# kawshik8/GAN-Image-Captioning

Hardware: AMD Instinct MI355X
Metric: captions/sec (G+D train step) (higher is better)
Workload: dtype bf16; 1 GPU; cfg2: adversarial G+D step, batch 64/GPU, 224x224 images, caption len 20, V=10000, E=H=512, 1-layer LSTM G, CNN-seq D (R=64,F=900), ResNet-50-shaped encoder, --conditional-gan 1; global_batch=64, caption_len=20, image_size=224, vocab=10000, conditional_gan=1, encoder=resnet50, step_impl=fused, parallelism=dp1

## Files before the change

gan-image-captioning_amd/_lib.py:

```python
from __future__ import annotations

import ctypes as C
import os

import torch

from . import build as _build

MAX_LAYERS = 4
MAX_CONVS = 8
F32, BF16 = 0, 1
LOSS_TYPES = {"standard": 0, "JS": 1, "KL": 2, "hinge": 3, "tv": 4, "rsgan": 5}

c_float_p = C.POINTER(C.c_float)
c_void_p = C.c_void_p


class DecoderDims(C.Structure):
    _fields_ = [(n, C.c_int32) for n in ("B", "L", "V", "E", "H", "NL", "dtype")]


class DecoderParams(C.Structure):
    _fields_ = [("embed", c_void_p), ("w_ih", c_void_p * MAX_LAYERS), ("w_hh", c_void_p * MAX_LAYERS),
                ("b_ih", c_void_p * MAX_LAYERS), ("b_hh", c_void_p * MAX_LAYERS), ("w_out", c_void_p), ("b_out", c_void_p)]
# ... 217 lines not shown
    "gic_repack_conv_weight": (C.c_int, [c_void_p, c_void_p, C.c_int, C.c_int, C.c_int, C.c_int, C.c_int, C.c_int, C.c_int, c_void_p]),
    "gic_conv2d_bn_in": (C.c_int, [c_void_p, c_void_p, C.c_int, c_void_p, c_void_p, C.c_float, c_void_p, c_void_p, c_void_p, C.c_int,
                         C.c_int] + [C.c_int] * 9 + [c_void_p]),
    "gic_conv1x1_res_in": (C.c_int, [c_void_p, c_void_p, C.c_int, c_void_p, c_void_p, c_void_p, c_void_p, C.c_int, c_void_p, c_void_p, C.c_float,
                           c_void_p, c_void_p, c_void_p, c_void_p, C.c_int, C.c_int, C.c_int, C.c_int, C.c_int, C.c_int, C.c_int, c_void_p]),
    "gic_conv1x1_bn_in_stats": (C.c_int, [c_void_p, c_void_p, C.c_int, c_void_p, c_void_p, C.c_float, c_void_p, c_void_p, C.c_int, C.c_int, C.c_int64,
                                C.c_int, C.c_int, c_void_p]),
    "gic_conv_b2b": (C.c_int, [c_void_p, c_void_p, C.c_int, c_void_p, c_void_p, c_void_p, c_void_p, C.c_int, c_void_p, c_void_p, c_void_p, c_void_p,
                     C.c_int, c_void_p, c_void_p, C.c_float, c_void_p, c_void_p, c_void_p, c_void_p, C.c_int, C.c_int, C.c_int64, C.c_int, C.c_int,
                     c_void_p]),
    "gic_conv_b2b_supported": (C.c_int, [C.c_int, C.c_int64, C.c_int, C.c_int]),
    "gic_conv2d": (C.c_int, [c_void_p, c_void_p, c_void_p, c_void_p, C.c_int, C.c_int] + [C.c_int] * 9 + [c_void_p]),
    "gic_bn_act": (C.c_int, [c_void_p] * 12 + [C.c_int, C.c_float, C.c_int, c_void_p, C.c_int, C.c_int64, C.c_int, c_void_p]),
    "gic_bn_relu_maxpool": (C.c_int, [c_void_p] * 6 + [C.c_int, C.c_float, c_void_p, C.c_int, C.c_int, C.c_int, C.c_int, C.c_int, c_void_p]),
    "gic_avgpool": (C.c_int, [c_void_p, c_void_p, C.c_int, C.c_int, C.c_int, C.c_int, c_void_p]),
    "gic_bn_running_update": (C.c_int, [c_void_p, C.c_int, c_void_p]),
    "gic_bn1d_fwd": (C.c_int, [c_void_p] * 5 + [C.c_int, C.c_float, C.c_float, c_void_p, c_void_p, c_void_p, C.c_int, C.c_int, c_void_p]),
    "gic_bn1d_bwd": (C.c_int, [c_void_p] * 4 + [C.c_int, c_void_p, c_void_p, c_void_p, C.c_int, C.c_int, c_void_p]),
    "gic_colsum": (C.c_int, [c_void_p, C.c_int, C.c_int64, C.c_int64, C.c_int64, c_void_p, C.c_int, c_void_p]),
    "gic_gan_losses": (C.c_int, [C.c_int, c_void_p, c_void_p, c_void_p, C.c_int64, c_void_p, c_void_p, c_void_p, c_void_p,
                                 c_void_p, c_void_p, c_void_p]),
    "gic_xent": (C.c_int, [c_void_p, C.c_int, C.c_int64, C.c_int32, c_void_p, c_void_p, c_void_p, c_void_p, c_void_p]),
    "gic_xent_seq": (C.c_int, [c_void_p, C.c_int, C.c_int64, C.c_int32, c_void_p, C.c_int64, c_void_p, C.c_int64, C.c_float, c_void_p, c_void_p,
                               c_void_p, c_void_p, c_void_p, c_void_p, c_void_p, c_void_p]),
    "gic_rollout_rewards": (C.c_int, [c_void_p, c_void_p, c_void_p, C.c_int, C.c_int, C.c_int, C.c_int, c_void_p]),
    "gic_cider_d": (C.c_int, [c_void_p, C.c_int64, c_void_p, c_void_p, C.c_int32, C.c_int32, c_void_p, C.c_int64, c_void_p, c_void_p,
                              C.c_int32, C.c_int32, C.c_int32, C.c_int32, c_void_p, c_void_p, C.c_int64, C.c_float, C.c_int32, c_void_p,
                              c_void_p]),
    "gic_caption_overlap": (C.c_int, [c_void_p, C.c_int64, c_void_p, c_void_p, C.c_int32, C.c_int32, c_void_p, C.c_int64, c_void_p, c_void_p,
                                      C.c_int32, C.c_int32, C.c_int32, C.c_int32, C.c_int32, c_void_p, c_void_p, c_void_p, c_void_p]),
# ... 60 lines not shown
```

gan-image-captioning_amd/csrc/encoder.hip:

```cpp
#include "../../include/gicap.h"
#include "kernels.h"
#include "bn_fold.h"
#include "conv_b2b.h"

namespace gic {
namespace {

template <typename TA, int PX>
__global__ __launch_bounds__(256) void pack_image_kernel(const float* __restrict__ img, TA* __restrict__ out, int N, int S, int pad, int Hp, int Wp) {
  const int groups = Wp / PX;
  const int total = N * Hp * groups;
  for (int i = blockIdx.x * blockDim.x + threadIdx.x; i < total; i += gridDim.x * blockDim.x) {
    const int gq = i % groups, t = i / groups;
    const int hp = t % Hp, n = t / Hp;
    const int h = hp - pad;
    const bool hok = h >= 0 && h < S;
    const int hc = min(max(h, 0), S - 1);
    float v[PX][3];
#pragma unroll
    for (int q = 0; q < PX; ++q) {
      const int w = gq * PX + q - pad;
      const int wc = min(max(w, 0), S - 1);
#pragma unroll
      for (int c = 0; c < 3; ++c) v[q][c] = img[(((long)n * 3 + c) * S + hc) * S + wc];
// ... 54 lines not shown
  shift = b.beta[c] - mean * scale;
}

__device__ __forceinline__ void stage_coeffs(float* coef, const BnSrc& b, int C, float inv_count) {
  for (int c = threadIdx.x; c < C; c += blockDim.x) {
    float sc, sh;
    bn_coeffs(b, c, C, inv_count, sc, sh);
    coef[c] = sc;
    coef[C + c] = sh;
  }
}

template <typename TA> struct Vec16 { static constexpr int N = 16 / sizeof(TA); };

template <typename TA, bool RES>
__global__ __launch_bounds__(1024) void bn_act_kernel(const TA* __restrict__ y, BnSrc by, const TA* __restrict__ res, BnSrc br,
                                                      float inv_count, int relu, TA* __restrict__ out, long rows, int C) {
  extern __shared__ __attribute__((aligned(16))) float coef[];
  constexpr int VN = Vec16<TA>::N;
  stage_coeffs(coef, by, C, inv_count);
  if (RES) stage_coeffs(coef + 2 * C, br, C, inv_count);
  __syncthreads();
  const int cv = C / VN;
  const long i0 = (long)blockIdx.x * blockDim.x + threadIdx.x;
  const int c0 = (int)(i0 % cv) * VN;
  float sc[VN], sh[VN], rs[VN], rh[VN];
#pragma unroll
  for (int k = 0; k < VN; ++k) {
    sc[k] = coef[c0 + k]; sh[k] = coef[C + c0 + k];
    rs[k] = RES ? coef[2 * C + c0 + k] : 0.f; rh[k] = RES ? coef[3 * C + c0 + k] : 0.f;
  }
  const long R = (long)gridDim.x * blockDim.x / cv;
  for (long r = i0 / cv; r < rows; r += 4 * R) {
    TA yv[4][VN], rv[4][VN];
    long o[4];
#pragma unroll
    for (int u = 0; u < 4; ++u) {
      const long ru = r + u * R;
      o[u] = (ru < rows ? ru : r) * C + c0;
      *(uint4*)yv[u] = *(const uint4*)(y + o[u]);
      if (RES) *(uint4*)rv[u] = *(const uint4*)(res + o[u]);
    }
#pragma unroll
    for (int u = 0; u < 4; ++u) {
      TA ov[VN];
#pragma unroll
      for (int k = 0; k < VN; ++k) {
        float v = to_f32<TA>(yv[u][k]) * sc[k] + sh[k];
        if (RES) v += to_f32<TA>(rv[u][k]) * rs[k] + rh[k];
        if (relu) v = fmaxf(v, 0.f);
        ov[k] = from_f32<TA>(v);
      }
      if (r + u * R < rows) *(uint4*)(out + o[u]) = *(const uint4*)ov;
    }
  }
}

template <typename TA>
__global__ __launch_bounds__(1024) void bn_relu_maxpool_kernel(const TA* __restrict__ y, BnSrc by, float inv_count, TA* __restrict__ out,
                                                                int N, int H, int W, int C, int Ho, int Wo) {
  extern __shared__ __attribute__((aligned(16))) float coef[];
  constexpr int VN = Vec16<TA>::N;
  stage_coeffs(coef, by, C, inv_count);
  __syncthreads();
  const int cv = C / VN;
  const long i0 = (long)blockIdx.x * blockDim.x + threadIdx.x;
  const int c0 = (int)(i0 % cv) * VN;
  float sc[VN], sh[VN];
#pragma unroll
// ... 33 lines not shown
  for (long i = (long)blockIdx.x * blockDim.x + threadIdx.x; i < total; i += (long)gridDim.x * blockDim.x) {
    const int c = (int)(i % C);
    const long n = i / C;
    const TA* xp = x + n * HW * C + c;
    float s = 0.f;
    int p = 0;
    for (; p + 7 <= HW; p += 7) {
      float v[7];
#pragma unroll
      for (int q = 0; q < 7; ++q) v[q] = to_f32<TA>(xp[(long)(p + q) * C]);
#pragma unroll
      for (int q = 0; q < 7; ++q) s += v[q];
    }
    for (; p < HW; ++p) s += to_f32<TA>(xp[(long)p * C]);
    out[i] = from_f32<TA>(s / (float)HW);
  }
}

__global__ void bn_running_update_kernel(const gic_bn_running_desc* __restrict__ table, int nlayers) {
  const int l = blockIdx.x;
  if (l >= nlayers) return;
  const gic_bn_running_desc d = table[l];
  const float inv = 1.f / d.count;
  const float unbias = d.count > 1.f ? d.count / (d.count - 1.f) : 1.f;
  for (int c = blockIdx.y * blockDim.x + threadIdx.x; c < d.C; c += blockDim.x * gridDim.y) {
    float s1 = 0.f, s2 = 0.f;
    for (int r = 0; r < d.nrep; ++r) { s1 += d.stats[(long)r * 2 * d.C + c]; s2 += d.stats[(long)r * 2 * d.C + d.C + c]; }
    const float mean = s1 * inv;
    const float var = fmaxf(s2 * inv - mean * mean, 0.f);
    d.running_mean[c] = (1.f - d.momentum) * d.running_mean[c] + d.momentum * mean;
// ... 59 lines not shown
  sg = bn1d_colsum(sg, red, r, c);
  sb = bn1d_colsum(sb, red, r, c);
  if (!live) return;
  if (r == 0) { dgamma[e] = sg; dbeta[e] = sb; }
  const float k = gamma[e] * invstd[e];
  const float invB = 1.f / (float)B;
  for (int b = r; b < B; b += 16) {
    const float d = dy[(long)b * E + e];
    dx[(long)b * E + e] = training ? k * (d - invB * (sb + xhat[(long)b * E + e] * sg)) : k * d;
  }
}

inline int grid1d(long total, int cap = 4096) {
  long g = (total + 255) / 256;
  return (int)(g < 1 ? 1 : (g > cap ? cap : g));
}
inline int bn_act_grid(long total) {
  long g = (total + 1023) / 1024;
  return (int)(g < 1 ? 1 : (g > 512 ? 512 : g));
}
inline int grid_periodic(long total, int period, int cap = 4096) {
  int g = grid1d(total, cap);
  const int mult = period > 256 ? period / 256 : 1;
  g = (g + mult - 1) / mult * mult;
  return g;
}

BnSrc make_src(const float* stats, int nrep, const float* gamma, const float* beta, const float* rm, const float* rv) {
  BnSrc s;
  s.stats = stats; s.nrep = nrep < 1 ? 1 : nrep; s.gamma = gamma; s.beta = beta; s.run_mean = rm; s.run_var = rv;
  return s;
}

GemmDesc conv_desc(const void* in, const void* w, void* out, float* stats, int stats_nrep, int dtype, int N, int H, int W, int Cin, int Cout,
// ... 123 lines not shown
  if (dtype != DT_BF16) return GIC_ERR_UNSUPPORTED;
  GemmDesc g = conv_desc(in, w, out, stats, stats_nrep, dtype, N, H, W, Cin, Cout, 1, 1, 1, 0);
  bn_on_load(g, in_stats, in_nrep, in_gamma, in_beta, count);
  g.res = res; g.res_stats = res_stats; g.res_nrep = res_nrep; g.res_gamma = res_gamma; g.res_beta = res_beta; g.res_inv_count = 1.f / count;
  g.out_wb = block_out;
  return gemm(g, (hipStream_t)stream);
}

int gic_bn_act(const void* y, const float* stats, const float* gamma, const float* beta, const float* run_mean, const float* run_var,
               const void* res, const float* res_stats, const float* res_gamma, const float* res_beta, const float* res_run_mean,
               const float* res_run_var, int stats_nrep, float count, int relu, void* out, int dtype, int64_t rows, int C, void* stream) {
  GIC_CHECK_ARG(y && out && gamma && beta && (stats || run_mean) && rows > 0 && count > 0, "bn_act: bad argument");
  const BnSrc by = make_src(stats, stats_nrep, gamma, beta, run_mean, run_var);
  const BnSrc br = make_src(res_stats, stats_nrep, res_gamma, res_beta, res_run_mean, res_run_var);
  GIC_CHECK_ARG(C % 8 == 0 && (C & (C - 1)) == 0, "bn_act: C must be a power of two >= 8 (got %d)", C);
  const size_t lds = (size_t)4 * C * sizeof(float);
  const int cv = C / (dtype == DT_F32 ? 4 : 8);
  const long total = rows * cv;
  int grid = bn_act_grid(total);
  {
    int step = cv, t = 1024;
    while (t) { const int m = step % t; step = t; t = m; }
    const int mult = cv / step;
    grid = (grid + mult - 1) / mult * mult;
    static const bool fit = getenv("GIC_BN_ACT_NO_FIT") == nullptr;
    if (fit && total > 4 * 1024) {
      const long rr = (rows + 3) / 4;
      long g = (rr * cv + 1023) / 1024;
      g = (g + mult - 1) / mult * mult;
      if (g <= 512) grid = (int)g;
    }
  }
  const hipStream_t st = (hipStream_t)stream;
  if (dtype == DT_F32) {
    if (res) hipLaunchKernelGGL((bn_act_kernel<float, true>), dim3(grid), dim3(1024), lds, st, (const float*)y, by, (const float*)res, br, 1.f / count, relu, (float*)out, (long)rows, C);
    else hipLaunchKernelGGL((bn_act_kernel<float, false>), dim3(grid), dim3(1024), lds, st, (const float*)y, by, (const float*)res, br, 1.f / count, relu, (float*)out, (long)rows, C);
  } else {
    if (res) hipLaunchKernelGGL((bn_act_kernel<bf16_t, true>), dim3(grid), dim3(1024), lds, st, (const bf16_t*)y, by, (const bf16_t*)res, br, 1.f / count, relu, (bf16_t*)out, (long)rows, C);
    else hipLaunchKernelGGL((bn_act_kernel<bf16_t, false>), dim3(grid), dim3(1024), lds, st, (const bf16_t*)y, by, (const bf16_t*)res, br, 1.f / count, relu, (bf16_t*)out, (long)rows, C);
  }
  GIC_CHECK_LAUNCH("bn_act");
  return GIC_OK;
}

int gic_bn_relu_maxpool(const void* y, const float* stats, const float* gamma, const float* beta, const float* run_mean,
                        const float* run_var, int stats_nrep, float count, void* out, int dtype, int N, int H, int W, int C, void* stream) {
  GIC_CHECK_ARG(y && out && gamma && beta && (stats || run_mean) && C % 8 == 0, "bn_relu_maxpool: bad argument");
  const int Ho = (H + 2 - 3) / 2 + 1, Wo = (W + 2 - 3) / 2 + 1;
  const BnSrc by = make_src(stats, stats_nrep, gamma, beta, run_mean, run_var);
  const size_t lds = (size_t)2 * C * sizeof(float);
  const int cv = C / (dtype == DT_F32 ? 4 : 8);
  const long total = (long)N * Ho * Wo * cv;
  GIC_CHECK_ARG((long)N * Ho * Wo < (1l << 31), "bn_relu_maxpool: too many output pixels");
  int grid = (int)((total + 1023) / 1024);
// ... 11 lines not shown
  GIC_CHECK_LAUNCH("bn_relu_maxpool");
  return GIC_OK;
}

int gic_avgpool(const void* x, void* out, int dtype, int N, int HW, int C, void* stream) {
  GIC_CHECK_ARG(x && out && N > 0 && HW > 0 && C > 0, "avgpool: bad argument");
  const long total = (long)N * C;
  if (dtype == DT_F32)
    hipLaunchKernelGGL((avgpool_kernel<float>), dim3(grid1d(total)), dim3(256), 0, (hipStream_t)stream, (const float*)x, (float*)out, N, HW, C);
  else
    hipLaunchKernelGGL((avgpool_kernel<bf16_t>), dim3(grid1d(total)), dim3(256), 0, (hipStream_t)stream, (const bf16_t*)x, (bf16_t*)out, N, HW, C);
  GIC_CHECK_LAUNCH("avgpool");
  return GIC_OK;
}

int gic_bn_running_update(const gic_bn_running_desc* table_dev, int nlayers, void* stream) {
  GIC_CHECK_ARG(table_dev && nlayers > 0, "bn_running_update: bad argument");
  hipLaunchKernelGGL(bn_running_update_kernel, dim3(nlayers, 8), dim3(256), 0, (hipStream_t)stream, table_dev, nlayers);
  GIC_CHECK_LAUNCH("bn_running_update");
  return GIC_OK;
}

int gic_bn1d_fwd(const float* x, const float* gamma, const float* beta, float* running_mean, float* running_var, int training,
                 float momentum, float eps, float* y, float* xhat, float* invstd, int B, int E, void* stream) {
  GIC_CHECK_ARG(x && gamma && beta && running_mean && running_var && y && xhat && invstd && B > 0 && E > 0, "bn1d_fwd: bad argument");
  hipLaunchKernelGGL(bn1d_fwd_kernel, dim3(cdiv(E, 16)), dim3(256), 0, (hipStream_t)stream, x, gamma, beta, running_mean, running_var,
                     training, momentum, eps, y, xhat, invstd, B, E);
  GIC_CHECK_LAUNCH("bn1d_fwd");
  return GIC_OK;
}
// ... 16 lines not shown
```

gan-image-captioning_amd/encoder_engine.py:

```python
from __future__ import annotations

import ctypes as C
import os
from typing import Dict, List, Optional, Tuple

import torch

from . import _lib as L
from . import engine
from .engine import ptr, stream_ptr

AVAILABLE = True
STATS_REPLICAS = 8


def _check(status, what):
    L.check(status, what)


class _NullCtx:
    def __enter__(self):
        return self

    def __exit__(self, *exc):
# ... 51 lines not shown
        off = 0
        for s in self.steps:
            s.stats_off = off
            off += 2 * s.cout * STATS_REPLICAS
        self.stats_len = off
        self._wkey = None
        self._bufs: Dict[Tuple[int, int], dict] = {}
        self._graphs: Dict[tuple, "torch.cuda.CUDAGraph"] = {}
        self._warm: set = set()
        self.fuse_in = not os.environ.get("GIC_NO_FUSED_BN_IN")
        self.fuse_res = os.environ.get("GIC_FUSED_RES_IN", "1") != "0"
        self.res_min_rows = int(os.environ.get("GIC_RES_IN_MIN_ROWS", "50000"))
        self.res_max_cout = int(os.environ.get("GIC_RES_IN_MAX_COUT", "128"))
        self.fuse_b2b = not os.environ.get("GIC_NO_CONV_B2B")
        self.b2b_only = int(os.environ.get("GIC_B2B_ONLY", "0"))
        self._nrep = {}
        self._det = False
        self.use_graph = not os.environ.get("GIC_NO_GRAPH")
        self.pending_tracked = 0
        self.conv_trace = None

    def sync_counters(self) -> None:
        if self.pending_tracked:
            for s in self.steps:
                s.bn.num_batches_tracked += self.pending_tracked
            self.pending_tracked = 0

    def _pack_weights(self, dev) -> None:
        key = (self.trunk._ptr_epoch, tuple(s.conv.weight._version for s in self.steps))
        if key == self._wkey:
# ... 198 lines not shown

    def _bn_args(self, s: Optional[_ConvStep], stats: Optional[torch.Tensor], training: bool):
        if s is None:
            return (None,) * 5
        g, b = ptr(s.bn.weight.detach()), ptr(s.bn.bias.detach())
        if training:
            return (stats.data_ptr() + 4 * s.stats_off, g, b, None, None)
        return (None, g, b, ptr(s.bn.running_mean), ptr(s.bn.running_var))

    def _bn_act(self, s, y, out, stats, training, rows, relu=True, res=None, res_step=None):
        a = self._bn_args(s, stats, training)
        r = self._bn_args(res_step, stats, training)
        _check(L.load().gic_bn_act(ptr(y), *a, ptr(res), *r, self._nrep[s.name], float(rows), int(relu), ptr(out), self.dtype, rows, s.cout, stream_ptr()),
               "gic_bn_act " + s.name)

    def forward(self, images: torch.Tensor, training: bool) -> torch.Tensor:
        engine.require_gpu(images)
        if images.dim() != 4 or images.shape[1] != 3 or images.shape[2] != images.shape[3] or images.dtype != torch.float32:
            raise ValueError(f"images must be float32 [N,3,S,S], got {tuple(images.shape)} {images.dtype}")
        N, S = images.shape[0], images.shape[2]
        if S % 2:
            raise ValueError("image size must be even")
        dev = images.device
        lib = L.load()
        self._det = engine.deterministic()
        self._cur = self._bkey(N, S)
        self._pack_weights(dev)
        b = self._buffers(N, S, dev)
        _check(lib.gic_pack_image(ptr(images.contiguous()), ptr(b["xin"]), self.dtype, N, S, 3, S + 6, stream_ptr()), "gic_pack_image")
        self._launch_trunk(b, N, S, training)
        if training:
            self.pending_tracked += 1
        return b["feat"]

    def last_map(self, N: int, S: int) -> torch.Tensor:
        return self._bufs[self._bkey(N, S)]["blocks"][-1]["out"]

    def _launch_trunk(self, b: dict, N: int, S: int, training: bool) -> None:
        if not self.use_graph:
            return self._run_trunk(b, N, S, training)
        key = (N, S, bool(training), self._det, self._wkey)
        g = self._graphs.get(key)
        if g is not None:
            g.replay()
        elif key not in self._warm:
            self._warm.add(key)
            self._run_trunk(b, N, S, training)
        else:
            self._graphs.clear()
            g = torch.cuda.CUDAGraph()
            try:
                with engine.capture_guard(), torch.cuda.graph(g, capture_error_mode="thread_local"):
                    self._run_trunk(b, N, S, training)
            except Exception as exc:
                import warnings
                warnings.warn(f"hipGraph capture of the trunk forward failed ({exc}); falling back to eager launches")
                self.use_graph = False
                torch.cuda.synchronize()
                return self._run_trunk(b, N, S, training)
            self._graphs[key] = g
            g.replay()

    def _run_trunk(self, b: dict, N: int, S: int, training: bool) -> None:
        lib = L.load()
        stats = b["stats"] if training else None
        if training:
            b["stats"].zero_()
        rows = b["rows"]
        self._conv(self.stem, b["xin"], b["y0"], stats, N, S + 6, S + 6, cin=4, kw=8, pad=0)
        h = b["y0"].shape[1]
        a = self._bn_args(self.stem, stats, training)
        _check(lib.gic_bn_relu_maxpool(ptr(b["y0"]), *a, self._nrep[self.stem.name], float(rows[self.stem.name]), ptr(b["x0"]), self.dtype, N, h, h, 64, stream_ptr()),
               "gic_bn_relu_maxpool")
        x = b["x0"]
        pend = None
        fuse_res = training and self.fuse_res and self.dtype != L.F32 and not self._det

        def flush():
            nonlocal pend
            if pend is not None:
                last, ylast, res, res_step, rows_, out = pend
                self._bn_act(last, ylast, out, stats, training, rows_, res=res, res_step=res_step)
                pend = None

        pend_b2b = None
        for bi, (blk, e) in enumerate(zip(self.blocks, b["blocks"])):
            c1, c2, c3, ds = blk["c1"], blk["c2"], blk["c3"], blk["ds"]
            hin, ho = e["hin"], e["hout"]
            nxt = self.blocks[bi + 1] if bi + 1 < len(self.blocks) else None
            b2b = False
            if blk["kind"] == "basic":
                flush()
                self._conv(c1, x, e["y1"], stats, N, hin, hin)
                self._bn_relu_conv(c1, e["y1"], e["z1"], c2, e["y2"], stats, training, N, ho, ho, rows[c1.name])
                last, ylast = c2, e["y2"]
            else:
                if pend_b2b is not None:
                    self._conv_b2b(pend_b2b, c1, e["y1"], stats)
                    pend_b2b = None
                elif pend is None or not self._conv1_res_in(pend, c1, e["y1"], stats, N, hin, hin):
                    flush()
                    self._conv(c1, x, e["y1"], stats, N, hin, hin)
                pend = None
                self._bn_relu_conv(c1, e["y1"], e["z1"], c2, e["y2"], stats, training, N, hin, hin, rows[c1.name])
                b2b = self._b2b_ok(blk, nxt, rows[c3.name], training) and self._conv3_stats_only(blk, e["y2"], stats, rows[c2.name], rows[c3.name])
                blk["b2b"] = bool(b2b)
                if not b2b:
                    self._bn_relu_conv(c2, e["y2"], e["z2"], c3, e["y3"], stats, training, N, ho, ho, rows[c2.name])
                last, ylast = c3, e["y3"]
            if ds is not None:
                self._conv(ds, x, e["yd"], stats, N, hin, hin)
                res, res_step = e["yd"], ds
            else:
                res, res_step = x, None
            if blk["kind"] != "basic" and b2b:
                pend_b2b = (c2, e["y2"], c3, res, res_step, rows[c3.name], e["out"])
            elif fuse_res and blk["kind"] != "basic":
                pend = (last, ylast, res, res_step, rows[last.name], e["out"])
            else:
                self._bn_act(last, ylast, e["out"], stats, training, rows[last.name], res=res, res_step=res_step)
            x = e["out"]
        flush()
        ho = x.shape[1]
        _check(lib.gic_avgpool(ptr(x), ptr(b["feat"]), self.dtype, N, ho * ho, x.shape[3], stream_ptr()), "gic_avgpool")
        if training:
            _check(lib.gic_bn_running_update(ptr(b["table"]), len(self.steps), stream_ptr()), "gic_bn_running_update")

    def replay(self, s: _ConvStep, xi, yo, stats, N: int, H: int, W: int, kw: dict, prev=None) -> None:
        if prev is not None and prev[0] == "b2b":
            self._conv_b2b(prev[1], s, yo, stats)
        elif prev is not None and prev[0] == "b2bstats":
            if not self._conv3_stats_only(prev[1], prev[2], stats, prev[3], prev[4]):
                raise RuntimeError("statistics-only conv3 refused for " + s.name)
        elif prev is not None and prev[0] == "res":
            if s.fused_in and self._conv1_res_in(prev[1], s, yo, stats, N, H, W):
                return
            self._conv(s, xi, yo, stats, N, H, W, **kw)
        elif prev is not None and s.fused_in:
            p, yp, rows_p = prev
# ... 156 lines not shown
```

gan-image-captioning_amd/generator.py:

```python
from __future__ import annotations

import math
from typing import List, Optional

import torch
import torch.nn as nn

from . import engine
from .trunk import ResNetTrunk, encoder_head_bwd, encoder_head_fwd


def _compute_dtype(args) -> int:
    return engine.parse_dtype(getattr(args, "compute_dtype", "bf16"))


class _SeedStream:

    def __init__(self):
        self._n = 0

    rank = 0

    def reset(self, n: int = 0) -> None:
        self._n = int(n)
# ... 520 lines not shown
                                   self.linear.weight, self.linear.bias, self.bn.weight, self.bn.bias,
                                   self.bn.running_mean, self.bn.running_var)
        return out, fmap.view(fmap.shape[0], -1, fmap.shape[-1])

    def prefetch_trunk(self, images, training: bool, after, mark=None, want_map: bool = False) -> None:
        if getattr(self, "_s_pre", None) is None:
            self._s_pre = torch.cuda.Stream(device=images.device)
        s = self._s_pre
        with engine.on_stream(s):
            s.wait_event(after)
            busy, self._busy = getattr(self, "_busy", None), None
            if busy is not None:
                s.wait_event(busy)
            if mark is not None:
                mark("trunk prefetch start [s_pre]", s)
            feats = self.trunk_features(images, training).clone()
            fmap = self.resnet._plan.last_map(images.shape[0], images.shape[2]).clone() if want_map else None
            done = s.record_event()
            if mark is not None:
                mark("trunk prefetch done [s_pre]", s)
        images.record_stream(s)
        self._pre = (images, bool(training), feats, done, fmap)

    def take_trunk(self, images, training: bool, stream):
        pre, self._pre = getattr(self, "_pre", None), None
        if pre is not None:
            stream.wait_event(pre[3])
            if pre[0] is images and pre[1] == bool(training):
                pre[2].record_stream(stream)
                return pre[2]
        busy = getattr(self, "_busy", None)
# ... 7 lines not shown
        pre, self._pre = getattr(self, "_pre", None), None
        if pre is not None:
            stream.wait_event(pre[3])
            if pre[0] is images and pre[1] == bool(training) and pre[4] is not None:
                pre[2].record_stream(stream)
                pre[4].record_stream(stream)
                return pre[2], pre[4]
        busy = getattr(self, "_busy", None)
        if busy is not None:
            stream.wait_event(busy)
        feats = self.trunk_features(images, training).clone()
        fmap = self.resnet._plan.last_map(images.shape[0], images.shape[2]).clone()
        self._busy = stream.record_event()
        return feats, fmap

    def trunk_features(self, images, training: bool):
        return self.resnet(images, _compute_dtype(self.args), training)

    def forward_fused(self, images, training: bool, trunk_feats=None):
        dt = _compute_dtype(self.args)
        feats = trunk_feats if trunk_feats is not None else self.resnet(images, dt, training)
        out, self._saved = encoder_head_fwd(dt, feats, self.linear.weight.detach(), self.linear.bias.detach(),
                                            self.bn.weight.detach(), self.bn.bias.detach(), self.bn.running_mean,
                                            self.bn.running_var, training, self.bn.momentum, self.bn.eps)
        return out

    def backward_fused(self, d_feat):
        grads = (self.linear.weight.grad, self.linear.bias.grad, self.bn.weight.grad, self.bn.bias.grad)
        encoder_head_bwd(_compute_dtype(self.args), self._saved, self.linear.weight.detach(), self.bn.weight.detach(), d_feat,
                         grads=grads)
        self._saved = None

# ... 96 lines not shown
```

gan-image-captioning_amd/trunk.py:

```python
from __future__ import annotations

from typing import Dict, List, Tuple

import torch
import torch.nn as nn

ARCHS = {
    "resnet18": ("basic", (2, 2, 2, 2), (64, 128, 256, 512), 1),
    "resnet50": ("bottleneck", (3, 4, 6, 3), (64, 128, 256, 512), 4),
}


class _ConvParams(nn.Module):
    def __init__(self, cin, cout, k, stride, pad):
        super().__init__()
        self.cin, self.cout, self.k, self.stride, self.pad = cin, cout, k, stride, pad
        w = torch.empty(cout, cin, k, k)
        nn.init.kaiming_normal_(w, mode="fan_out", nonlinearity="relu")
        self.weight = nn.Parameter(w)


class _BNParams(nn.Module):
    def __init__(self, c):
        super().__init__()
# ... 45 lines not shown
        self._plan = None
        self._ptr_epoch = 0
        self.register_load_state_dict_post_hook(lambda module, incompatible: module._bump_ptr_epoch())

    def _bump_ptr_epoch(self) -> None:
        self._ptr_epoch += 1

    def _apply(self, fn, *args, **kwargs):
        out = super()._apply(fn, *args, **kwargs)
        self._ptr_epoch += 1
        return out

    def stages(self) -> List[nn.Sequential]:
        return [getattr(self, str(i)) for i in (4, 5, 6, 7)]

    def forward(self, images: torch.Tensor, dtype: int, training=None) -> torch.Tensor:
        from . import encoder_engine
        if self._plan is None or self._plan.dtype != dtype:
            self._plan = encoder_engine.TrunkPlan(self, dtype)
        return self._plan.forward(images, self.training if training is None else training)

    def state_dict(self, *a, **k):
        if self._plan is not None:
            self._plan.sync_counters()
        return super().state_dict(*a, **k)


def encoder_head_fwd(dtype, feat, weight, bias, gamma, beta, running_mean, running_var, training, momentum, eps):
    from . import encoder_engine
    return encoder_engine.head_fwd(dtype, feat, weight, bias, gamma, beta, running_mean, running_var, training, momentum, eps)


def encoder_head_bwd(dtype, saved, weight, gamma, d_out, grads=None):
    from . import encoder_engine
    return encoder_engine.head_bwd(dtype, saved, weight, gamma, d_out, grads=grads)
# ... 1 lines not shown
```

include/gicap.h:

```cpp
#ifndef GICAP_H_
#define GICAP_H_

#include <stdint.h>

#ifdef __cplusplus
extern "C" {
#endif

#define GIC_ABI_VERSION 5
#define GIC_MAX_LAYERS 4
#define GIC_MAX_CONVS 8

enum gic_status {
  GIC_STATUS_OK = 0,
  GIC_STATUS_INVALID_ARG = -1,
  GIC_STATUS_UNSUPPORTED = -2,
  GIC_STATUS_LAUNCH = -3,
  GIC_STATUS_WORKSPACE = -4
};
enum gic_dtype { GIC_F32 = 0, GIC_BF16 = 1 };
enum gic_loss_type {
  GIC_LOSS_STANDARD = 0, GIC_LOSS_JS = 1, GIC_LOSS_KL = 2, GIC_LOSS_HINGE = 3, GIC_LOSS_TV = 4, GIC_LOSS_RSGAN = 5
};

// ... 403 lines not shown
int gic_conv1x1_bn_in_stats(const void* in, const float* in_stats, int in_nrep, const float* in_gamma, const float* in_beta, float in_count,
                            const void* w, float* stats, int stats_nrep, int dtype, int64_t rows, int Cin, int Cout, void* stream);
int gic_conv_b2b(const void* y2, const float* stats2, int nrep2, const float* gamma2, const float* beta2, const void* w3, const float* stats3,
                 int nrep3, const float* gamma3, const float* beta3, const void* res, const float* res_stats, int res_nrep,
                 const float* res_gamma, const float* res_beta, float count, void* block_out, const void* w1n, void* y1n, float* stats1,
                 int nrep1, int dtype, int64_t rows, int C2, int C1N, void* stream);
int gic_conv_b2b_supported(int dtype, int64_t rows, int C2, int C1N);
int gic_bn_act(const void* y, const float* stats, const float* gamma, const float* beta, const float* run_mean,
               const float* run_var, const void* res, const float* res_stats, const float* res_gamma, const float* res_beta,
               const float* res_run_mean, const float* res_run_var, int stats_nrep, float count, int relu, void* out, int dtype,
               int64_t rows, int C, void* stream);
int gic_bn_relu_maxpool(const void* y, const float* stats, const float* gamma, const float* beta, const float* run_mean,
                        const float* run_var, int stats_nrep, float count, void* out, int dtype, int N, int H, int W, int C,
                        void* stream);
int gic_avgpool(const void* x, void* out, int dtype, int N, int HW, int C, void* stream);
typedef struct gic_bn_running_desc {
  const float* stats;
  float* running_mean;
  float* running_var;
  float count;
  float momentum;
  int32_t C;
  int32_t nrep;
} gic_bn_running_desc;
int gic_bn_running_update(const gic_bn_running_desc* table_dev, int nlayers, void* stream);
int gic_bn1d_fwd(const float* x, const float* gamma, const float* beta, float* running_mean, float* running_var, int training,
                 float momentum, float eps, float* y, float* xhat, float* invstd, int B, int E, void* stream);
int gic_bn1d_bwd(const float* dy, const float* xhat, const float* invstd, const float* gamma, int training, float* dx,
                 float* dgamma, float* dbeta, int B, int E, void* stream);
int gic_colsum(const void* A, int dtype, int64_t lda, int64_t rows, int64_t cols, float* out, int accumulate, void* stream);
// ... 42 lines not shown
```

Baseline: 26930 captions/s.

## Fuse final BN-activation with average pooling and retile bn_act kernel

Adds a bn_act_avgpool kernel that applies the last block's BN, residual and ReLU, stages the result in LDS, and reduces it to pooled features in the same pass. Writing the full feature map becomes optional when the caller does not need it. This removes a separate avgpool pass and its reread of the map. The generic bn_act kernel is also reworked to use 256-thread blocks over 64-channel groups, computing only per-group coefficients and issuing the next loads before the current tile is processed. The cost is new plumbing through trunk, generator and graph keys, plus a fallback path when LDS is too small.

```diff
diff --git a/gan-image-captioning_amd/_lib.py b/gan-image-captioning_amd/_lib.py
--- a/gan-image-captioning_amd/_lib.py
+++ b/gan-image-captioning_amd/_lib.py
@@ -255,6 +255,7 @@
     "gic_bn_act": (C.c_int, [c_void_p] * 12 + [C.c_int, C.c_float, C.c_int, c_void_p, C.c_int, C.c_int64, C.c_int, c_void_p]),
     "gic_bn_relu_maxpool": (C.c_int, [c_void_p] * 6 + [C.c_int, C.c_float, c_void_p, C.c_int, C.c_int, C.c_int, C.c_int, C.c_int, c_void_p]),
     "gic_avgpool": (C.c_int, [c_void_p, c_void_p, C.c_int, C.c_int, C.c_int, C.c_int, c_void_p]),
+    "gic_bn_act_avgpool": (C.c_int, [c_void_p] * 12 + [C.c_int, C.c_float, C.c_int, c_void_p, c_void_p, C.c_int, C.c_int, C.c_int, C.c_int, c_void_p]),
     "gic_bn_running_update": (C.c_int, [c_void_p, C.c_int, c_void_p]),
     "gic_bn1d_fwd": (C.c_int, [c_void_p] * 5 + [C.c_int, C.c_float, C.c_float, c_void_p, c_void_p, c_void_p, C.c_int, C.c_int, c_void_p]),
     "gic_bn1d_bwd": (C.c_int, [c_void_p] * 4 + [C.c_int, c_void_p, c_void_p, c_void_p, C.c_int, C.c_int, c_void_p]),
diff --git a/gan-image-captioning_amd/csrc/encoder.hip b/gan-image-captioning_amd/csrc/encoder.hip
--- a/gan-image-captioning_amd/csrc/encoder.hip
+++ b/gan-image-captioning_amd/csrc/encoder.hip
@@ -92,45 +92,65 @@
 template <typename TA> struct Vec16 { static constexpr int N = 16 / sizeof(TA); };
 
 template <typename TA, bool RES>
-__global__ __launch_bounds__(1024) void bn_act_kernel(const TA* __restrict__ y, BnSrc by, const TA* __restrict__ res, BnSrc br,
-                                                      float inv_count, int relu, TA* __restrict__ out, long rows, int C) {
-  extern __shared__ __attribute__((aligned(16))) float coef[];
+__device__ __forceinline__ TA bn_act_elem(TA yv, TA rv, float sc, float sh, float rs, float rh, int relu) {
+  float v = to_f32<TA>(yv) * sc + sh;
+  if (RES) v += to_f32<TA>(rv) * rs + rh;
+  if (relu) v = fmaxf(v, 0.f);
+  return from_f32<TA>(v);
+}
+
+constexpr int kBnActCG = 64;
+template <typename TA, bool RES>
+__global__ __launch_bounds__(256) void bn_act_kernel(const TA* __restrict__ y, BnSrc by, const TA* __restrict__ res, BnSrc br,
+                                                     float inv_count, int relu, TA* __restrict__ out, long rows, int C, int CG) {
+  __shared__ float coef[4 * kBnActCG];
   constexpr int VN = Vec16<TA>::N;
-  stage_coeffs(coef, by, C, inv_count);
-  if (RES) stage_coeffs(coef + 2 * C, br, C, inv_count);
-  __syncthreads();
-  const int cv = C / VN;
-  const long i0 = (long)blockIdx.x * blockDim.x + threadIdx.x;
-  const int c0 = (int)(i0 % cv) * VN;
-  float sc[VN], sh[VN], rs[VN], rh[VN];
-#pragma unroll
-  for (int k = 0; k < VN; ++k) {
-    sc[k] = coef[c0 + k]; sh[k] = coef[C + c0 + k];
-    rs[k] = RES ? coef[2 * C + c0 + k] : 0.f; rh[k] = RES ? coef[3 * C + c0 + k] : 0.f;
-  }
-  const long R = (long)gridDim.x * blockDim.x / cv;
-  for (long r = i0 / cv; r < rows; r += 4 * R) {
-    TA yv[4][VN], rv[4][VN];
-    long o[4];
+  const int lanes = CG / VN, slots = 256 / lanes, groups = C / CG;
+  const int g = blockIdx.x % groups;
+  const long chunk = blockIdx.x / groups, nchunk = gridDim.x / groups;
+  const int cl = (threadIdx.x % lanes) * VN, slot = threadIdx.x / lanes;
+  const long col = (long)g * CG + cl;
+  {
+    const int t = threadIdx.x;
+    float a, b;
+    if (t < CG) {
+      bn_coeffs(by, g * CG + t, C, inv_count, a, b);
+      coef[t] = a; coef[CG + t] = b;
+    } else if (RES && t < 2 * CG) {
+      bn_coeffs(br, g * CG + t - CG, C, inv_count, a, b);
+      coef[2 * CG + t - CG] = a; coef[3 * CG + t - CG] = b;
+    }
+  }
+  long r = chunk * (4 * slots) + slot;
+  TA yv[4][VN], rv[4][VN];
+  long o[4];
+  auto issue = [&](long r_) {
 #pragma unroll
     for (int u = 0; u < 4; ++u) {
-      const long ru = r + u * R;
-      o[u] = (ru < rows ? ru : r) * C + c0;
+      const long ru = r_ + (long)u * slots;
+      o[u] = (ru < rows ? ru : rows - 1) * C + col;
       *(uint4*)yv[u] = *(const uint4*)(y + o[u]);
       if (RES) *(uint4*)rv[u] = *(const uint4*)(res + o[u]);
     }
+  };
+  issue(r);
+  __syncthreads();
+  float sc[VN], sh[VN], rs[VN], rh[VN];
+#pragma unroll
+  for (int k = 0; k < VN; ++k) {
+    sc[k] = coef[cl + k]; sh[k] = coef[CG + cl + k];
+    rs[k] = RES ? coef[2 * CG + cl + k] : 0.f; rh[k] = RES ? coef[3 * CG + cl + k] : 0.f;
+  }
+  while (r < rows) {
 #pragma unroll
     for (int u = 0; u < 4; ++u) {
       TA ov[VN];
 #pragma unroll
-      for (int k = 0; k < VN; ++k) {
-        float v = to_f32<TA>(yv[u][k]) * sc[k] + sh[k];
-        if (RES) v += to_f32<TA>(rv[u][k]) * rs[k] + rh[k];
-        if (relu) v = fmaxf(v, 0.f);
-        ov[k] = from_f32<TA>(v);
-      }
-      if (r + u * R < rows) *(uint4*)(out + o[u]) = *(const uint4*)ov;
-    }
+      for (int k = 0; k < VN; ++k) ov[k] = bn_act_elem<TA, RES>(yv[u][k], rv[u][k], sc[k], sh[k], rs[k], rh[k], relu);
+      if (r + (long)u * slots < rows) *(uint4*)(out + o[u]) = *(const uint4*)ov;
+    }
+    r += nchunk * (4 * slots);
+    if (r < rows) issue(r);
   }
 }
 
@@ -194,6 +214,80 @@
     }
     for (; p < HW; ++p) s += to_f32<TA>(xp[(long)p * C]);
     out[i] = from_f32<TA>(s / (float)HW);
+  }
+}
+
+constexpr int kPoolCG = 64;
+template <typename TA, bool RES>
+__global__ __launch_bounds__(256) void bn_act_avgpool_kernel(const TA* __restrict__ y, BnSrc by, const TA* __restrict__ res, BnSrc br,
+                                                              float inv_count, int relu, TA* __restrict__ out, TA* __restrict__ pooled,
+                                                              int HW, int C) {
+  extern __shared__ __attribute__((aligned(16))) float pool_lds[];
+  constexpr int VN = Vec16<TA>::N, CG = kPoolCG, CV = CG / VN, SLOTS = 256 / CV;
+  float* coef = pool_lds;
+  TA* tile = (TA*)(pool_lds + 4 * CG);
+  const int groups = C / CG;
+  const int g = blockIdx.x % groups;
+  const long n = blockIdx.x / groups;
+  const int cl = (threadIdx.x % CV) * VN;
+  const int slot = threadIdx.x / CV;
+  const long base = n * HW * C + g * CG + cl;
+  TA yv[2][VN], rv[2][VN];
+  auto issue = [&](int p0) {
+#pragma unroll
+    for (int u = 0; u < 2; ++u) {
+      const int p = min(p0 + slot + u * SLOTS, HW - 1);
+      *(uint4*)yv[u] = *(const uint4*)(y + base + (long)p * C);
+      if (RES) *(uint4*)rv[u] = *(const uint4*)(res + base + (long)p * C);
+    }
+  };
+  {
+    const int t = threadIdx.x;
+    float a, b;
+    if (t < CG) {
+      bn_coeffs(by, g * CG + t, C, inv_count, a, b);
+      coef[t] = a; coef[CG + t] = b;
+    } else if (RES && t < 2 * CG) {
+      bn_coeffs(br, g * CG + t - CG, C, inv_count, a, b);
+      coef[2 * CG + t - CG] = a; coef[3 * CG + t - CG] = b;
+    }
+  }
+  issue(0);
+  __syncthreads();
+  float sc[VN], sh[VN], rs[VN], rh[VN];
+#pragma unroll
+  for (int k = 0; k < VN; ++k) {
+    sc[k] = coef[cl + k]; sh[k] = coef[CG + cl + k];
+    rs[k] = RES ? coef[2 * CG + cl + k] : 0.f; rh[k] = RES ? coef[3 * CG + cl + k] : 0.f;
+  }
+  for (int p0 = 0; p0 < HW; p0 += 2 * SLOTS) {
+#pragma unroll
+    for (int u = 0; u < 2; ++u) {
+      const int p = p0 + slot + u * SLOTS;
+      TA ov[VN];
+#pragma unroll
+      for (int k = 0; k < VN; ++k) ov[k] = bn_act_elem<TA, RES>(yv[u][k], rv[u][k], sc[k], sh[k], rs[k], rh[k], relu);
+      if (p < HW) {
+        *(uint4*)(tile + p * CG + cl) = *(const uint4*)ov;
+        if (out) *(uint4*)(out + base + (long)p * C) = *(const uint4*)ov;
+      }
+    }
+    if (p0 + 2 * SLOTS < HW) issue(p0 + 2 * SLOTS);
+  }
+  __syncthreads();
+  if (threadIdx.x < CG) {
+    const TA* tp = tile + threadIdx.x;
+    float s = 0.f;
+    int p = 0;
+    for (; p + 7 <= HW; p += 7) {
+      float v[7];
+#pragma unroll
+      for (int q = 0; q < 7; ++q) v[q] = to_f32<TA>(tp[(p + q) * CG]);
+#pragma unroll
+      for (int q = 0; q < 7; ++q) s += v[q];
+    }
+    for (; p < HW; ++p) s += to_f32<TA>(tp[p * CG]);
+    pooled[n * C + g * CG + threadIdx.x] = from_f32<TA>(s / (float)HW);
   }
 }
 
@@ -283,10 +377,6 @@
 inline int grid1d(long total, int cap = 4096) {
   long g = (total + 255) / 256;
   return (int)(g < 1 ? 1 : (g > cap ? cap : g));
-}
-inline int bn_act_grid(long total) {
-  long g = (total + 1023) / 1024;
-  return (int)(g < 1 ? 1 : (g > 512 ? 512 : g));
 }
 inline int grid_periodic(long total, int period, int cap = 4096) {
   int g = grid1d(total, cap);
@@ -440,30 +530,21 @@
   const BnSrc by = make_src(stats, stats_nrep, gamma, beta, run_mean, run_var);
   const BnSrc br = make_src(res_stats, stats_nrep, res_gamma, res_beta, res_run_mean, res_run_var);
   GIC_CHECK_ARG(C % 8 == 0 && (C & (C - 1)) == 0, "bn_act: C must be a power of two >= 8 (got %d)", C);
-  const size_t lds = (size_t)4 * C * sizeof(float);
-  const int cv = C / (dtype == DT_F32 ? 4 : 8);
-  const long total = rows * cv;
-  int grid = bn_act_grid(total);
-  {
-    int step = cv, t = 1024;
-    while (t) { const int m = step % t; step = t; t = m; }
-    const int mult = cv / step;
-    grid = (grid + mult - 1) / mult * mult;
-    static const bool fit = getenv("GIC_BN_ACT_NO_FIT") == nullptr;
-    if (fit && total > 4 * 1024) {
-      const long rr = (rows + 3) / 4;
-      long g = (rr * cv + 1023) / 1024;
-      g = (g + mult - 1) / mult * mult;
-      if (g <= 512) grid = (int)g;
-    }
-  }
+  const int CG = C < kBnActCG ? C : kBnActCG;
+  const int lanes = CG / (dtype == DT_F32 ? 4 : 8), slots = 256 / lanes, groups = C / CG;
+  const long chunks = (rows + 4 * slots - 1) / (4 * slots);
+  const long cap = groups < 2048 ? 2048 / groups : 1;
+  const long trips = (chunks + cap - 1) / cap;
+  const long nchunk = (chunks + trips - 1) / trips;
+  const dim3 grid((unsigned)(groups * nchunk)), block(256);
   const hipStream_t st = (hipStream_t)stream;
+  const float ic = 1.f / count;
   if (dtype == DT_F32) {
-    if (res) hipLaunchKernelGGL((bn_act_kernel<float, true>), dim3(grid), dim3(1024), lds, st, (const float*)y, by, (const float*)res, br, 1.f / count, relu, (float*)out, (long)rows, C);
-    else hipLaunchKernelGGL((bn_act_kernel<float, false>), dim3(grid), dim3(1024), lds, st, (const float*)y, by, (const float*)res, br, 1.f / count, relu, (float*)out, (long)rows, C);
+    if (res) hipLaunchKernelGGL((bn_act_kernel<float, true>), grid, block, 0, st, (const float*)y, by, (const float*)res, br, ic, relu, (float*)out, (long)rows, C, CG);
+    else hipLaunchKernelGGL((bn_act_kernel<float, false>), grid, block, 0, st, (const float*)y, by, (const float*)res, br, ic, relu, (float*)out, (long)rows, C, CG);
   } else {
-    if (res) hipLaunchKernelGGL((bn_act_kernel<bf16_t, true>), dim3(grid), dim3(1024), lds, st, (const bf16_t*)y, by, (const bf16_t*)res, br, 1.f / count, relu, (bf16_t*)out, (long)rows, C);
-    else hipLaunchKernelGGL((bn_act_kernel<bf16_t, false>), dim3(grid), dim3(1024), lds, st, (const bf16_t*)y, by, (const bf16_t*)res, br, 1.f / count, relu, (bf16_t*)out, (long)rows, C);
+    if (res) hipLaunchKernelGGL((bn_act_kernel<bf16_t, true>), grid, block, 0, st, (const bf16_t*)y, by, (const bf16_t*)res, br, ic, relu, (bf16_t*)out, (long)rows, C, CG);
+    else hipLaunchKernelGGL((bn_act_kernel<bf16_t, false>), grid, block, 0, st, (const bf16_t*)y, by, (const bf16_t*)res, br, ic, relu, (bf16_t*)out, (long)rows, C, CG);
   }
   GIC_CHECK_LAUNCH("bn_act");
   return GIC_OK;
@@ -505,6 +586,31 @@
   return GIC_OK;
 }
 
+int gic_bn_act_avgpool(const void* y, const float* stats, const float* gamma, const float* beta, const float* run_mean, const float* run_var,
+                       const void* res, const float* res_stats, const float* res_gamma, const float* res_beta, const float* res_run_mean,
+                       const float* res_run_var, int stats_nrep, float count, int relu, void* out, void* pooled, int dtype, int N, int HW,
+                       int C, void* stream) {
+  GIC_CHECK_ARG(y && pooled && gamma && beta && (stats || run_mean) && N > 0 && HW > 0 && count > 0, "bn_act_avgpool: bad argument");
+  GIC_CHECK_ARG(C > 0 && C % kPoolCG == 0, "bn_act_avgpool: C must be a multiple of %d (got %d)", kPoolCG, C);
+  const size_t esz = dtype == DT_F32 ? 4 : 2;
+  const size_t lds = (size_t)4 * kPoolCG * sizeof(float) + (size_t)HW * kPoolCG * esz;
+  const long blocks = (long)N * (C / kPoolCG);
+  if (lds > 64 * 1024 || blocks >= (1l << 31)) return GIC_ERR_UNSUPPORTED;
+  const BnSrc by = make_src(stats, stats_nrep, gamma, beta, run_mean, run_var);
+  const BnSrc br = make_src(res_stats, stats_nrep, res_gamma, res_beta, res_run_mean, res_run_var);
+  const hipStream_t st = (hipStream_t)stream;
+  const float ic = 1.f / count;
+  if (dtype == DT_F32) {
+    if (res) hipLaunchKernelGGL((bn_act_avgpool_kernel<float, true>), dim3((int)blocks), dim3(256), lds, st, (const float*)y, by, (const float*)res, br, ic, relu, (float*)out, (float*)pooled, HW, C);
+    else hipLaunchKernelGGL((bn_act_avgpool_kernel<float, false>), dim3((int)blocks), dim3(256), lds, st, (const float*)y, by, (const float*)res, br, ic, relu, (float*)out, (float*)pooled, HW, C);
+  } else {
+    if (res) hipLaunchKernelGGL((bn_act_avgpool_kernel<bf16_t, true>), dim3((int)blocks), dim3(256), lds, st, (const bf16_t*)y, by, (const bf16_t*)res, br, ic, relu, (bf16_t*)out, (bf16_t*)pooled, HW, C);
+    else hipLaunchKernelGGL((bn_act_avgpool_kernel<bf16_t, false>), dim3((int)blocks), dim3(256), lds, st, (const bf16_t*)y, by, (const bf16_t*)res, br, ic, relu, (bf16_t*)out, (bf16_t*)pooled, HW, C);
+  }
+  GIC_CHECK_LAUNCH("bn_act_avgpool");
+  return GIC_OK;
+}
+
 int gic_bn_running_update(const gic_bn_running_desc* table_dev, int nlayers, void* stream) {
   GIC_CHECK_ARG(table_dev && nlayers > 0, "bn_running_update: bad argument");
   hipLaunchKernelGGL(bn_running_update_kernel, dim3(nlayers, 8), dim3(256), 0, (hipStream_t)stream, table_dev, nlayers);
diff --git a/gan-image-captioning_amd/encoder_engine.py b/gan-image-captioning_amd/encoder_engine.py
--- a/gan-image-captioning_amd/encoder_engine.py
+++ b/gan-image-captioning_amd/encoder_engine.py
@@ -89,6 +89,7 @@
         self.res_max_cout = int(os.environ.get("GIC_RES_IN_MAX_COUT", "128"))
         self.fuse_b2b = not os.environ.get("GIC_NO_CONV_B2B")
         self.b2b_only = int(os.environ.get("GIC_B2B_ONLY", "0"))
+        self.fuse_pool = not os.environ.get("GIC_NO_FUSED_AVGPOOL")
         self._nrep = {}
         self._det = False
         self.use_graph = not os.environ.get("GIC_NO_GRAPH")
@@ -317,7 +318,7 @@
         _check(L.load().gic_bn_act(ptr(y), *a, ptr(res), *r, self._nrep[s.name], float(rows), int(relu), ptr(out), self.dtype, rows, s.cout, stream_ptr()),
                "gic_bn_act " + s.name)
 
-    def forward(self, images: torch.Tensor, training: bool) -> torch.Tensor:
+    def forward(self, images: torch.Tensor, training: bool, want_map: bool = True) -> torch.Tensor:
         engine.require_gpu(images)
         if images.dim() != 4 or images.shape[1] != 3 or images.shape[2] != images.shape[3] or images.dtype != torch.float32:
             raise ValueError(f"images must be float32 [N,3,S,S], got {tuple(images.shape)} {images.dtype}")
@@ -331,7 +332,7 @@
         self._pack_weights(dev)
         b = self._buffers(N, S, dev)
         _check(lib.gic_pack_image(ptr(images.contiguous()), ptr(b["xin"]), self.dtype, N, S, 3, S + 6, stream_ptr()), "gic_pack_image")
-        self._launch_trunk(b, N, S, training)
+        self._launch_trunk(b, N, S, training, want_map)
         if training:
             self.pending_tracked += 1
         return b["feat"]
@@ -339,32 +340,32 @@
     def last_map(self, N: int, S: int) -> torch.Tensor:
         return self._bufs[self._bkey(N, S)]["blocks"][-1]["out"]
 
-    def _launch_trunk(self, b: dict, N: int, S: int, training: bool) -> None:
+    def _launch_trunk(self, b: dict, N: int, S: int, training: bool, want_map: bool = True) -> None:
         if not self.use_graph:
-            return self._run_trunk(b, N, S, training)
-        key = (N, S, bool(training), self._det, self._wkey)
+            return self._run_trunk(b, N, S, training, want_map)
+        key = (N, S, bool(training), self._det, self._wkey, bool(want_map) or not self.fuse_pool)
         g = self._graphs.get(key)
         if g is not None:
             g.replay()
         elif key not in self._warm:
             self._warm.add(key)
-            self._run_trunk(b, N, S, training)
+            self._run_trunk(b, N, S, training, want_map)
         else:
             self._graphs.clear()
             g = torch.cuda.CUDAGraph()
             try:
                 with engine.capture_guard(), torch.cuda.graph(g, capture_error_mode="thread_local"):
-                    self._run_trunk(b, N, S, training)
+                    self._run_trunk(b, N, S, training, want_map)
             except Exception as exc:
                 import warnings
                 warnings.warn(f"hipGraph capture of the trunk forward failed ({exc}); falling back to eager launches")
                 self.use_graph = False
                 torch.cuda.synchronize()
-                return self._run_trunk(b, N, S, training)
+                return self._run_trunk(b, N, S, training, want_map)
             self._graphs[key] = g
             g.replay()
 
-    def _run_trunk(self, b: dict, N: int, S: int, training: bool) -> None:
+    def _run_trunk(self, b: dict, N: int, S: int, training: bool, want_map: bool = True) -> None:
         lib = L.load()
         stats = b["stats"] if training else None
         if training:
@@ -386,6 +387,7 @@
                 self._bn_act(last, ylast, out, stats, training, rows_, res=res, res_step=res_step)
                 pend = None
 
+        tail = None
         pend_b2b = None
         for bi, (blk, e) in enumerate(zip(self.blocks, b["blocks"])):
             c1, c2, c3, ds = blk["c1"], blk["c2"], blk["c3"], blk["ds"]
@@ -416,16 +418,29 @@
                 res, res_step = e["yd"], ds
             else:
                 res, res_step = x, None
-            if blk["kind"] != "basic" and b2b:
+            if nxt is None and self.fuse_pool:
+                tail = (last, ylast, res, res_step, rows[last.name], e["out"])
+            elif blk["kind"] != "basic" and b2b:
                 pend_b2b = (c2, e["y2"], c3, res, res_step, rows[c3.name], e["out"])
             elif fuse_res and blk["kind"] != "basic":
                 pend = (last, ylast, res, res_step, rows[last.name], e["out"])
             else:
                 self._bn_act(last, ylast, e["out"], stats, training, rows[last.name], res=res, res_step=res_step)
             x = e["out"]
-        flush()
         ho = x.shape[1]
-        _check(lib.gic_avgpool(ptr(x), ptr(b["feat"]), self.dtype, N, ho * ho, x.shape[3], stream_ptr()), "gic_avgpool")
+        if tail is not None:
+            last, ylast, res, res_step, rows_, out = tail
+            status = lib.gic_bn_act_avgpool(ptr(ylast), *self._bn_args(last, stats, training), ptr(res), *self._bn_args(res_step, stats, training),
+                                            self._nrep[last.name], float(rows_), 1, ptr(out) if want_map else None, ptr(b["feat"]), self.dtype,
+                                            N, ho * ho, last.cout, stream_ptr())
+            if status != L.ERR_UNSUPPORTED:
+                _check(status, "gic_bn_act_avgpool " + last.name)
+                tail = None
+            else:
+                pend = tail
+        if tail is not None or not self.fuse_pool:
+            flush()
+            _check(lib.gic_avgpool(ptr(x), ptr(b["feat"]), self.dtype, N, ho * ho, x.shape[3], stream_ptr()), "gic_avgpool")
         if training:
             _check(lib.gic_bn_running_update(ptr(b["table"]), len(self.steps), stream_ptr()), "gic_bn_running_update")
 
diff --git a/gan-image-captioning_amd/generator.py b/gan-image-captioning_amd/generator.py
--- a/gan-image-captioning_amd/generator.py
+++ b/gan-image-captioning_amd/generator.py
@@ -558,7 +558,7 @@
                 s.wait_event(busy)
             if mark is not None:
                 mark("trunk prefetch start [s_pre]", s)
-            feats = self.trunk_features(images, training).clone()
+            feats = self.trunk_features(images, training, want_map).clone()
             fmap = self.resnet._plan.last_map(images.shape[0], images.shape[2]).clone() if want_map else None
             done = s.record_event()
             if mark is not None:
@@ -596,8 +596,8 @@
         self._busy = stream.record_event()
         return feats, fmap
 
-    def trunk_features(self, images, training: bool):
-        return self.resnet(images, _compute_dtype(self.args), training)
+    def trunk_features(self, images, training: bool, want_map: bool = True):
+        return self.resnet(images, _compute_dtype(self.args), training, want_map)
 
     def forward_fused(self, images, training: bool, trunk_feats=None):
         dt = _compute_dtype(self.args)
diff --git a/gan-image-captioning_amd/trunk.py b/gan-image-captioning_amd/trunk.py
--- a/gan-image-captioning_amd/trunk.py
+++ b/gan-image-captioning_amd/trunk.py
@@ -83,11 +83,11 @@
     def stages(self) -> List[nn.Sequential]:
         return [getattr(self, str(i)) for i in (4, 5, 6, 7)]
 
-    def forward(self, images: torch.Tensor, dtype: int, training=None) -> torch.Tensor:
+    def forward(self, images: torch.Tensor, dtype: int, training=None, want_map: bool = True) -> torch.Tensor:
         from . import encoder_engine
         if self._plan is None or self._plan.dtype != dtype:
             self._plan = encoder_engine.TrunkPlan(self, dtype)
-        return self._plan.forward(images, self.training if training is None else training)
+        return self._plan.forward(images, self.training if training is None else training, want_map)
 
     def state_dict(self, *a, **k):
         if self._plan is not None:
diff --git a/include/gicap.h b/include/gicap.h
--- a/include/gicap.h
+++ b/include/gicap.h
@@ -441,6 +441,10 @@
                         const float* run_var, int stats_nrep, float count, void* out, int dtype, int N, int H, int W, int C,
                         void* stream);
 int gic_avgpool(const void* x, void* out, int dtype, int N, int HW, int C, void* stream);
+int gic_bn_act_avgpool(const void* y, const float* stats, const float* gamma, const float* beta, const float* run_mean,
+                       const float* run_var, const void* res, const float* res_stats, const float* res_gamma, const float* res_beta,
+                       const float* res_run_mean, const float* res_run_var, int stats_nrep, float count, int relu, void* out,
+                       void* pooled, int dtype, int N, int HW, int C, void* stream);
 typedef struct gic_bn_running_desc {
   const float* stats;
   float* running_mean;
```

Result: no change. 26910 captions/s, median of 2 (-0.1%).
